# SitaoLuan/When-Do-GNNs-Help

Measured on AMD Instinct MI355X. Metric: aggregation edges/sec (whole job; + %HBM roofline of the SpMM kernel), higher is better.
Workload: dtype f32; 1 GPU; synthetic homophily sweep (data_synthesis/4000-equivalent): 10 h-levels x 5 seeds = 50 graphs/GPU/step, N=2000 nodes, k=10, F=500 fp32, C=5; step = batched D^-1(A+I)X aggregation + edge/label stati...; parallelism=independent sweep shards x1 (no data-path collective; job-table broadcast + r...

## Files before the change

when-do-gnns-help_amd/csrc/gemm.hip:

```cpp
#include "wdg_common.h"
#include "split_bf16.h"

namespace {

using namespace wdg;

typedef float f32x16 __attribute__((ext_vector_type(16)));

constexpr int BM = 128, BK = 16, THREADS = 256;
constexpr int LDA_S = BK + 1;

template <int NT>
__device__ __forceinline__ void tile_bias(global_ptr<const float> bias, int col0, int li, int N, float (&bv)[NT]) {
#pragma unroll
    for (int t = 0; t < NT; ++t) {
        const int gn = col0 + t * 32 + li;
        bv[t] = (bias && gn < N) ? bias[gn] : 0.f;
    }
}

template <int NT>
__device__ __forceinline__ void tile_store(const f32x16 (&acc)[NT], float (&bv)[NT], global_ptr<float> C, int64_t ldc, int row0,
                                           int col0, int li, int lk, int M, int N, int act) {
#pragma unroll
    for (int t = 0; t < NT; ++t) asm volatile("" : "+v"(bv[t]));
    const bool relu = act == WDG_ACT_RELU;
    const bool full = row0 + 32 <= M;
#pragma unroll
    for (int t = 0; t < NT; ++t) {
        const int gn = col0 + t * 32 + li;
        if (gn >= N) continue;
        global_ptr<float> p = C + static_cast<int64_t>(row0 + 4 * lk) * ldc + gn;
#pragma unroll
        for (int r = 0; r < 16; ++r) {
            float v = acc[t][r] + bv[t];
            if (relu) v = fmaxf(v, 0.f);
            if (full || row0 + (r & 3) + 8 * (r >> 2) + 4 * lk < M) *p = v;
            p += ((r & 3) == 3) ? 5 * ldc : ldc;
            if ((r & 3) == 3) __builtin_amdgcn_sched_barrier(0);
        }
    }
}

template <int NT, bool TRANSB>
__global__ __launch_bounds__(THREADS) void gemm_f32_kernel(const wdg_gemm_job *__restrict__ jobs,
                                                           const wdg_gemm_job inline_job) {
    constexpr int BN = 32 * NT;
    constexpr int LDB_S = TRANSB ? (BK + 1) : (BN + 1);
    __shared__ float As[BM * LDA_S];
    __shared__ float Bs[TRANSB ? BN * LDB_S : BK * LDB_S];

    const desc_ptr<wdg_gemm_job> job = descriptor(jobs, inline_job, blockIdx.z);
    const global_ptr<const float> A = to_global(job->A), B = to_global(job->B), bias = to_global(job->bias);
    const global_ptr<float> C = to_global(job->C);
    const int64_t lda = job->lda, ldb = job->ldb, ldc = job->ldc;
    const int M = job->M, N = job->N, K = job->K, act = job->act;
    const int tid = threadIdx.x, wave = tid >> 6, lane = tid & 63;
    const int m0 = blockIdx.x * BM, n0 = blockIdx.y * BN;
    if (m0 >= M || n0 >= N) return;
    const bool split = jobs == nullptr && gridDim.z > 1;
    int kb = 0, ke = K;
    global_ptr<float> Cw = C;
    if (split) {
        const int kc = (((K + static_cast<int>(gridDim.z) - 1) / static_cast<int>(gridDim.z)) + BK - 1) / BK * BK;
        kb = min(K, static_cast<int>(blockIdx.z) * kc), ke = min(K, kb + kc);
        Cw = C + static_cast<int64_t>(blockIdx.z) * M * ldc;
    }

    constexpr int A_PER = BM * BK / THREADS;
    constexpr int B_PER = BN * BK / THREADS;
    float ra[A_PER], rb[B_PER];

    auto load_tiles = [&](int k0) {
#pragma unroll
        for (int i = 0; i < A_PER; ++i) {
            const int e = tid + i * THREADS, k = e % BK, m = e / BK;
            const int gm = m0 + m, gk = k0 + k;
            ra[i] = (gm < M && gk < ke) ? A[static_cast<int64_t>(gm) * lda + gk] : 0.f;
        }
#pragma unroll
        for (int i = 0; i < B_PER; ++i) {
            const int e = tid + i * THREADS;
            if constexpr (TRANSB) {
                const int k = e % BK, n = e / BK;
                const int gn = n0 + n, gk = k0 + k;
                rb[i] = (gn < N && gk < ke) ? B[static_cast<int64_t>(gn) * ldb + gk] : 0.f;
            } else {
                const int n = e % BN, k = e / BN;
                const int gn = n0 + n, gk = k0 + k;
                rb[i] = (gn < N && gk < ke) ? B[static_cast<int64_t>(gk) * ldb + gn] : 0.f;
            }
        }
    };
    auto store_tiles = [&]() {
#pragma unroll
        for (int i = 0; i < A_PER; ++i) {
            const int e = tid + i * THREADS, k = e % BK, m = e / BK;
            As[m * LDA_S + k] = ra[i];
        }
#pragma unroll
        for (int i = 0; i < B_PER; ++i) {
            const int e = tid + i * THREADS;
            if constexpr (TRANSB) {
                const int k = e % BK, n = e / BK;
                Bs[n * LDB_S + k] = rb[i];
            } else {
                const int n = e % BN, k = e / BN;
                Bs[k * LDB_S + n] = rb[i];
            }
        }
    };

    f32x16 acc[NT];
#pragma unroll
    for (int t = 0; t < NT; ++t)
#pragma unroll
        for (int r = 0; r < 16; ++r) acc[t][r] = 0.f;

    const int li = lane & 31, lk = lane >> 5;
    float bv[NT];
    tile_bias<NT>(bias, n0, li, N, bv);
    load_tiles(kb);
    for (int k0 = kb; k0 < ke; k0 += BK) {
        __syncthreads();
        store_tiles();
        __syncthreads();
        if (k0 + BK < ke) load_tiles(k0 + BK);
#pragma unroll
        for (int kk = 0; kk < BK; kk += 2) {
            const float a = As[(wave * 32 + li) * LDA_S + kk + lk];
#pragma unroll
            for (int t = 0; t < NT; ++t) {
                float b;
                if constexpr (TRANSB) b = Bs[(t * 32 + li) * LDB_S + kk + lk];
                else b = Bs[(kk + lk) * LDB_S + t * 32 + li];
                acc[t] = __builtin_amdgcn_mfma_f32_32x32x2f32(a, b, acc[t], 0, 0, 0);
            }
        }
    }

    tile_store<NT>(acc, bv, Cw, ldc, m0 + wave * 32, n0, li, lk, M, N, act);
}

__global__ __launch_bounds__(256) void gemm_splitk_reduce(const float *__restrict__ P, int splits, int M, int N, int64_t ldp,
                                                          const float *__restrict__ bias, int act, float *__restrict__ C, int64_t ldc) {
    const int64_t i = static_cast<int64_t>(blockIdx.x) * 256 + threadIdx.x;
    if (i >= static_cast<int64_t>(M) * N) return;
    const int m = static_cast<int>(i / N), n = static_cast<int>(i % N);
    float v = P[static_cast<int64_t>(m) * ldp + n];
    for (int z = 1; z < splits; ++z) v += P[(static_cast<int64_t>(z) * M + m) * ldp + n];
    if (bias) v += bias[n];
    if (act == WDG_ACT_RELU) v = fmaxf(v, 0.f);
    C[static_cast<int64_t>(m) * ldc + n] = v;
}

constexpr int BRES_THREADS = 1024, BRES_COLS = 64;

struct BresGroup {
    f32x4_t r[4];
};

template <int NT, bool SWAP>
__device__ __forceinline__ void bres_compute(const BresGroup &grp, int kbase, int lk, int li, const float *Bres,
                                             f32x16 (&acc)[NT]) {
    float lo[8], hi[8];
#pragma unroll
    for (int j = 0; j < 4; ++j) {
        const auto xy = __builtin_amdgcn_permlane32_swap(__float_as_uint(grp.r[j].x), __float_as_uint(grp.r[j].y), false, false);
        const auto zw = __builtin_amdgcn_permlane32_swap(__float_as_uint(grp.r[j].z), __float_as_uint(grp.r[j].w), false, false);
        lo[2 * j] = __uint_as_float(xy[0]), hi[2 * j] = __uint_as_float(xy[1]);
        lo[2 * j + 1] = __uint_as_float(zw[0]), hi[2 * j + 1] = __uint_as_float(zw[1]);
    }
    constexpr int CH = 2, CHUNKS = 16 / CH;
    float bq[2][CH][NT];
    auto read_chunk = [&](int c, float (&dst)[CH][NT]) {
#pragma unroll
        for (int s = 0; s < CH; ++s) {
            const int row = kbase + 2 * (CH * c + s) + lk;
#pragma unroll
            for (int t = 0; t < NT; ++t) dst[s][t] = Bres[row * BRES_COLS + ((t * 32 + li) ^ (lk << 5))];
        }
    };
    read_chunk(0, bq[0]);
#pragma unroll
    for (int c = 0; c < CHUNKS; ++c) {
        if (c + 1 < CHUNKS) read_chunk(c + 1, bq[(c + 1) & 1]);
        __builtin_amdgcn_sched_barrier(0);
#pragma unroll
        for (int s = 0; s < CH; ++s) {
            const int h = CH * c + s;
            const float a = h < 8 ? lo[h] : hi[h - 8];
#pragma unroll
            for (int t = 0; t < NT; ++t)
                acc[t] = SWAP ? __builtin_amdgcn_mfma_f32_32x32x2f32(bq[c & 1][s][t], a, acc[t], 0, 0, 0)
                              : __builtin_amdgcn_mfma_f32_32x32x2f32(a, bq[c & 1][s][t], acc[t], 0, 0, 0);
        }
        __builtin_amdgcn_sched_barrier(0);
    }
}

__device__ __forceinline__ void bres_stage_b(global_ptr<const float> B, int64_t ldb, int K, int N, float *Bres) {
    const int k_rows = (K + 31) / 32 * 32;
    for (int base = threadIdx.x; base < k_rows * BRES_COLS; base += 8 * BRES_THREADS) {
        float v[8];
#pragma unroll
        for (int u = 0; u < 8; ++u) {
            const int idx = base + u * BRES_THREADS, k = idx / BRES_COLS, n = idx % BRES_COLS;
            v[u] = (k < K && n < N) ? B[static_cast<int64_t>(k) * ldb + n] : 0.f;
        }
#pragma unroll
        for (int u = 0; u < 8; ++u) {
            const int idx = base + u * BRES_THREADS, k = idx / BRES_COLS;
            if (idx < k_rows * BRES_COLS) Bres[idx ^ ((k & 1) << 5)] = v[u];
        }
    }
}

template <int NT, bool SWAP>
__device__ __forceinline__ void bres_tile(global_ptr<const float> a_lane, int K, int lk, int li, const float *Bres,
                                          f32x16 (&acc)[NT]) {
    const int full = K / 32;
    BresGroup g0, g1;
    auto load_group = [&](int g, BresGroup &dst) {
#pragma unroll
        for (int j = 0; j < 4; ++j) dst.r[j] = *(const global_ptr<const f32x4_t>)(a_lane + g * 32 + j * 4);
    };
    int g = 0;
    if (full > 0) load_group(0, g0);
    for (; g + 2 <= full; g += 2) {
        load_group(g + 1, g1);
        __builtin_amdgcn_sched_barrier(0);
        bres_compute<NT, SWAP>(g0, g * 32, lk, li, Bres, acc);
        __builtin_amdgcn_sched_barrier(0);
        load_group(min(g + 2, full - 1), g0);
        __builtin_amdgcn_sched_barrier(0);
        bres_compute<NT, SWAP>(g1, (g + 1) * 32, lk, li, Bres, acc);
        __builtin_amdgcn_sched_barrier(0);
    }
    if (g < full) bres_compute<NT, SWAP>(g0, g * 32, lk, li, Bres, acc), ++g;
    if (full * 32 < K) {
#pragma unroll
        for (int j = 0; j < 4; ++j) {
            const int k0 = full * 32 + 16 * lk + j * 4;
            g1.r[j] = f32x4_t{0.f, 0.f, 0.f, 0.f};
            if (k0 < K) g1.r[j] = *(const global_ptr<const f32x4_t>)(a_lane + full * 32 + j * 4);
        }
        bres_compute<NT, SWAP>(g1, full * 32, lk, li, Bres, acc);
    }
}

template <int NT>
__global__ __launch_bounds__(BRES_THREADS) void gemm_bres_kernel(const wdg_gemm_job *__restrict__ jobs,
                                                                   const wdg_gemm_job inline_job, int n_parts) {
    extern __shared__ float Bres[];
    const int job_id = blockIdx.x / n_parts, part = blockIdx.x % n_parts;
    const desc_ptr<wdg_gemm_job> job = descriptor(jobs, inline_job, job_id);
    const global_ptr<const float> A = to_global(job->A), B = to_global(job->B), bias = to_global(job->bias);
    const global_ptr<float> C = to_global(job->C);
    const int64_t lda = job->lda, ldb = job->ldb, ldc = job->ldc;
    const int M = job->M, N = job->N, K = job->K, act = job->act;
    const int wave = threadIdx.x >> 6, lane = threadIdx.x & 63, li = lane & 31, lk = lane >> 5;
    if (M <= 0 || N <= 0) return;
    bres_stage_b(B, ldb, K, N, Bres);
    __syncthreads();

    const int tiles = (M + 31) / 32, per_part = (tiles + n_parts - 1) / n_parts;
    const int t_end = min((part + 1) * per_part, tiles);
    for (int tile = part * per_part + wave; tile < t_end; tile += BRES_THREADS / 64) {
        const int gm = tile * 32 + li;
        const global_ptr<const float> a_lane = A + static_cast<int64_t>(gm < M ? gm : M - 1) * lda + 16 * lk;
        f32x16 acc[NT];
#pragma unroll
        for (int t = 0; t < NT; ++t)
#pragma unroll
            for (int r = 0; r < 16; ++r) acc[t][r] = 0.f;
        float bv[NT];
        tile_bias<NT>(bias, 0, li, N, bv);
        bres_tile<NT, false>(a_lane, K, lk, li, Bres, acc);
        tile_store<NT>(acc, bv, C, ldc, tile * 32, 0, li, lk, M, N, act);
    }
}

constexpr int MLP2_MAX_C = 8;

template <int NT>
__global__ __launch_bounds__(BRES_THREADS) void mlp2_bres_kernel(const wdg_mlp2_job *__restrict__ jobs, int n_parts) {
    extern __shared__ float Bres[];
    const int job_id = blockIdx.x / n_parts, part = blockIdx.x % n_parts;
    const desc_ptr<wdg_mlp2_job> job = (desc_ptr<wdg_mlp2_job>)(jobs + job_id);
    const global_ptr<const float> A = to_global(job->A), W0 = to_global(job->W0), b0 = to_global(job->b0);
    const global_ptr<const float> W1 = to_global(job->W1), b1 = to_global(job->b1);
    const global_ptr<float> Z = to_global(job->Z);
    const int64_t lda = job->lda, ldw0 = job->ldw0, ldw1 = job->ldw1, ldz = job->ldz;
    const int M = job->M, K = job->K, H = job->H, C = job->C, act = job->act;
    const int wave = threadIdx.x >> 6, lane = threadIdx.x & 63, li = lane & 31, lk = lane >> 5;
    if (M <= 0 || H <= 0 || C <= 0) return;
    float *const w1s = Bres + (K + 31) / 32 * 32 * BRES_COLS;
    float *const b0s = w1s + BRES_COLS * MLP2_MAX_C;
    bres_stage_b(W0, ldw0, K, H, Bres);
    for (int idx = threadIdx.x; idx < BRES_COLS * MLP2_MAX_C; idx += BRES_THREADS) {
        const int col = idx / MLP2_MAX_C, c = idx % MLP2_MAX_C;
        w1s[idx] = (col < H && c < C) ? W1[static_cast<int64_t>(col) * ldw1 + c] : 0.f;
    }
    if (threadIdx.x < BRES_COLS) b0s[threadIdx.x] = (b0 && threadIdx.x < H) ? b0[threadIdx.x] : 0.f;
    __syncthreads();

    const int tiles = (M + 31) / 32, per_part = (tiles + n_parts - 1) / n_parts;
    const int t_end = min((part + 1) * per_part, tiles);
    const bool relu = act == WDG_ACT_RELU;
    for (int tile = part * per_part + wave; tile < t_end; tile += BRES_THREADS / 64) {
        const int gm = tile * 32 + li;
        const global_ptr<const float> a_lane = A + static_cast<int64_t>(gm < M ? gm : M - 1) * lda + 16 * lk;
        f32x16 acc[NT];
#pragma unroll
        for (int t = 0; t < NT; ++t)
#pragma unroll
            for (int r = 0; r < 16; ++r) acc[t][r] = 0.f;
        bres_tile<NT, true>(a_lane, K, lk, li, Bres, acc);

        float z[MLP2_MAX_C];
#pragma unroll
        for (int c = 0; c < MLP2_MAX_C; ++c) z[c] = 0.f;
        int lds_off = lk * 4;
        asm volatile("" : "+v"(lds_off));
#pragma unroll
        for (int t = 0; t < NT; ++t) {
#pragma unroll
            for (int r4 = 0; r4 < 4; ++r4) {
                const int col0 = t * 32 + r4 * 8 + lds_off;
                const float4 bb = *reinterpret_cast<const float4 *>(b0s + col0);
                float h[4] = {acc[t][4 * r4] + bb.x, acc[t][4 * r4 + 1] + bb.y, acc[t][4 * r4 + 2] + bb.z, acc[t][4 * r4 + 3] + bb.w};
#pragma unroll
                for (int e = 0; e < 4; ++e) {
                    if (relu) h[e] = fmaxf(h[e], 0.f);
                    const float4 wa = *reinterpret_cast<const float4 *>(w1s + (col0 + e) * MLP2_MAX_C);
                    const float4 wb = *reinterpret_cast<const float4 *>(w1s + (col0 + e) * MLP2_MAX_C + 4);
                    z[0] = fmaf(h[e], wa.x, z[0]); z[1] = fmaf(h[e], wa.y, z[1]);
                    z[2] = fmaf(h[e], wa.z, z[2]); z[3] = fmaf(h[e], wa.w, z[3]);
                    z[4] = fmaf(h[e], wb.x, z[4]); z[5] = fmaf(h[e], wb.y, z[5]);
                    z[6] = fmaf(h[e], wb.z, z[6]); z[7] = fmaf(h[e], wb.w, z[7]);
                }
                __builtin_amdgcn_sched_barrier(0);
            }
        }
#pragma unroll
        for (int c = 0; c < MLP2_MAX_C; ++c) z[c] += __shfl_xor(z[c], 32);
        if (lk == 0 && gm < M) {
            const global_ptr<float> zp = Z + static_cast<int64_t>(gm) * ldz;
#pragma unroll
            for (int c = 0; c < MLP2_MAX_C; ++c)
                if (c < C) zp[c] = z[c] + (b1 ? b1[c] : 0.f);
        }
    }
}

constexpr int SPLIT_KQ = 128, SPLIT_KB = SPLIT_KQ / 8;
constexpr int SPLIT_PIECE_WORDS = SPLIT_KB * BRES_COLS * 4;
constexpr int SPLIT_BUF_WORDS = 3 * SPLIT_PIECE_WORDS;
static_assert(SPLIT_KB * BRES_COLS == BRES_THREADS, "one (k block, column) pair of a buffer per thread");

__device__ __forceinline__ void split_load_w(global_ptr<const float> W0, int64_t ldw0, int K, int H, int k0, float (&w)[8]) {
    int tid = threadIdx.x;
    asm volatile("" : "+v"(tid));
    const int col = tid % BRES_COLS, kb = tid / BRES_COLS;
    if (k0 + SPLIT_KQ <= K && H == BRES_COLS) {
        const global_ptr<const float> p = W0 + static_cast<int64_t>(k0 + 8 * kb) * ldw0 + col;
#pragma unroll
        for (int j = 0; j < 8; ++j) w[j] = p[j * ldw0];
        return;
    }
#pragma unroll
    for (int j = 0; j < 8; ++j) {
        const int k = k0 + 8 * kb + j;
        const float v = W0[static_cast<int64_t>(min(k, K - 1)) * ldw0 + min(col, H - 1)];
        w[j] = (k < K && col < H) ? v : 0.f;
    }
}
__device__ __forceinline__ void split_write_w(const float (&w)[8], unsigned *buf) {
    unsigned h[4], m[4], l[4];
#pragma unroll
    for (int j = 0; j < 4; ++j) split_pair(w[2 * j], w[2 * j + 1], h[j], m[j], l[j]);
    u32x4_t *dst = reinterpret_cast<u32x4_t *>(buf) + threadIdx.x;
    dst[0] = u32x4_t{h[0], h[1], h[2], h[3]};
    dst[SPLIT_PIECE_WORDS / 4] = u32x4_t{m[0], m[1], m[2], m[3]};
    dst[2 * (SPLIT_PIECE_WORDS / 4)] = u32x4_t{l[0], l[1], l[2], l[3]};
}

typedef float f32x4_acc __attribute__((ext_vector_type(4)));
struct SplitStep { f32x4_t a[2], b[2]; };

template <int NT16>
__device__ __forceinline__ void split_compute(const SplitStep &c, int kb, int n, const unsigned *Ws, f32x4_acc (&acc)[2][NT16]) {
    u32x4_t xh[2], xm[2], xl[2];
#pragma unroll
    for (int s = 0; s < 2; ++s) {
        unsigned ph[4], pm[4], pl[4];
        split_pair(c.a[s].x, c.a[s].y, ph[0], pm[0], pl[0]);
        split_pair(c.a[s].z, c.a[s].w, ph[1], pm[1], pl[1]);
        split_pair(c.b[s].x, c.b[s].y, ph[2], pm[2], pl[2]);
        split_pair(c.b[s].z, c.b[s].w, ph[3], pm[3], pl[3]);
        xh[s] = u32x4_t{ph[0], ph[1], ph[2], ph[3]}, xm[s] = u32x4_t{pm[0], pm[1], pm[2], pm[3]}, xl[s] = u32x4_t{pl[0], pl[1], pl[2], pl[3]};
    }
    const u32x4_t *wrow = reinterpret_cast<const u32x4_t *>(Ws) + kb * BRES_COLS + n;
#pragma unroll
    for (int T = 0; T < NT16; ++T) {
        const u32x4_t wl = wrow[T * 16 + 2 * (SPLIT_PIECE_WORDS / 4)];
        const u32x4_t wm = wrow[T * 16 + SPLIT_PIECE_WORDS / 4];
        const u32x4_t wh = wrow[T * 16];
#pragma unroll
        for (int s = 0; s < 2; ++s) {
            acc[s][T] = __builtin_amdgcn_mfma_f32_16x16x32_bf16(as_frag(wl), as_frag(xh[s]), acc[s][T], 0, 0, 0);
            acc[s][T] = __builtin_amdgcn_mfma_f32_16x16x32_bf16(as_frag(wm), as_frag(xm[s]), acc[s][T], 0, 0, 0);
            acc[s][T] = __builtin_amdgcn_mfma_f32_16x16x32_bf16(as_frag(wm), as_frag(xh[s]), acc[s][T], 0, 0, 0);
            acc[s][T] = __builtin_amdgcn_mfma_f32_16x16x32_bf16(as_frag(wh), as_frag(xl[s]), acc[s][T], 0, 0, 0);
            acc[s][T] = __builtin_amdgcn_mfma_f32_16x16x32_bf16(as_frag(wh), as_frag(xm[s]), acc[s][T], 0, 0, 0);
            acc[s][T] = __builtin_amdgcn_mfma_f32_16x16x32_bf16(as_frag(wh), as_frag(xh[s]), acc[s][T], 0, 0, 0);
        }
    }
}

template <int NT>
__global__ __launch_bounds__(BRES_THREADS) void mlp2_split_kernel(const wdg_mlp2_job *__restrict__ jobs, int n_parts) {
    constexpr int NT16 = 2 * NT;
    extern __shared__ float Bres[];
    const int job_id = blockIdx.x / n_parts, part = blockIdx.x % n_parts;
    const desc_ptr<wdg_mlp2_job> job = (desc_ptr<wdg_mlp2_job>)(jobs + job_id);
    const global_ptr<const float> A = to_global(job->A), W0 = to_global(job->W0), b0 = to_global(job->b0);
    const global_ptr<const float> W1 = to_global(job->W1), b1 = to_global(job->b1);
    const global_ptr<float> Z = to_global(job->Z);
    const int64_t lda = job->lda, ldw0 = job->ldw0, ldw1 = job->ldw1, ldz = job->ldz;
    const int64_t ags = job->a_group_stride > 0 ? job->a_group_stride : 16;
    const int M = job->M, K = job->K, H = job->H, C = job->C, act = job->act;
    const int wave = threadIdx.x >> 6, lane = threadIdx.x & 63, n = lane & 15, q = lane >> 4;
    if (M <= 0 || H <= 0 || C <= 0) return;
    unsigned *const Ws = reinterpret_cast<unsigned *>(Bres);
    float *const w1s = Bres + 2 * SPLIT_BUF_WORDS;
    float *const b0s = w1s + BRES_COLS * MLP2_MAX_C;
    for (int idx = threadIdx.x; idx < BRES_COLS * MLP2_MAX_C; idx += BRES_THREADS) {
        const int col = idx / MLP2_MAX_C, c = idx % MLP2_MAX_C;
        w1s[idx] = (col < H && c < C) ? W1[static_cast<int64_t>(col) * ldw1 + c] : 0.f;
    }
    if (threadIdx.x < BRES_COLS) b0s[threadIdx.x] = (b0 && threadIdx.x < H) ? b0[threadIdx.x] : 0.f;

    const int tiles = (M + 31) / 32, per_part = (tiles + n_parts - 1) / n_parts;
    const int t_first = part * per_part, t_end = min((part + 1) * per_part, tiles);
    const bool relu = act == WDG_ACT_RELU;
    const int steps = (K + 31) / 32, quarters = (K + SPLIT_KQ - 1) / SPLIT_KQ;
    for (int t0 = t_first; t0 < t_end; t0 += BRES_THREADS / 64) {
        const int tile = t0 + wave;
        const bool have = tile < t_end;
        global_ptr<const float> a_row[2];
#pragma unroll
        for (int s = 0; s < 2; ++s) {
            const int gm = tile * 32 + 16 * s + n;
            a_row[s] = A + static_cast<int64_t>(have && gm < M ? gm : M - 1) * lda + (q >> 1) * ags + (q & 1) * 8;
        }
        f32x4_acc acc[2][NT16];
#pragma unroll
        for (int s = 0; s < 2; ++s)
#pragma unroll
            for (int T = 0; T < NT16; ++T) acc[s][T] = f32x4_acc{0.f, 0.f, 0.f, 0.f};
        auto load_step = [&](int st, SplitStep &dst) {
            st = min(st, steps - 1);
            if (32 * st + 32 <= K) {
#pragma unroll
                for (int s = 0; s < 2; ++s) {
                    dst.a[s] = *(const global_ptr<const f32x4_t>)(a_row[s] + 2 * ags * st);
                    dst.b[s] = *(const global_ptr<const f32x4_t>)(a_row[s] + 2 * ags * st + 4);
                }
                return;
            }
            const int k = 32 * st + 8 * q;
            const f32x4_t zero{0.f, 0.f, 0.f, 0.f};
#pragma unroll
            for (int s = 0; s < 2; ++s) {
                const global_ptr<const float> row0 = a_row[s] - ((q >> 1) * ags + (q & 1) * 8);
                const int ka = min(k, K - 4), kb = min(k + 4, K - 4);
                const f32x4_t va = *(const global_ptr<const f32x4_t>)(row0 + (ka >> 4) * ags + (ka & 15));
                const f32x4_t vb = *(const global_ptr<const f32x4_t>)(row0 + (kb >> 4) * ags + (kb & 15));
                dst.a[s] = k < K ? va : zero;
                dst.b[s] = k + 4 < K ? vb : zero;
            }
        };
        SplitStep sa, sb;
        float w[8];
        load_step(0, sa);
        split_load_w(W0, ldw0, K, H, 0, w);
        split_write_w(w, Ws);
        __syncthreads();
        for (int qu = 0; qu < quarters; ++qu) {
            const unsigned *cur = Ws + (qu & 1) * SPLIT_BUF_WORDS;
            if (qu + 1 < quarters) split_load_w(W0, ldw0, K, H, (qu + 1) * SPLIT_KQ, w);
            if (have) {
#pragma unroll
                for (int c = 0; c < 4; c += 2) {
                    const int base = 4 * qu + c;
                    if (base >= steps) break;
                    load_step(base + 1, sb);
                    __builtin_amdgcn_sched_barrier(0);
                    split_compute<NT16>(sa, 4 * c + q, n, cur, acc);
                    __builtin_amdgcn_sched_barrier(0);
                    load_step(base + 2, sa);
                    __builtin_amdgcn_sched_barrier(0);
                    if (base + 1 < steps) split_compute<NT16>(sb, 4 * c + 4 + q, n, cur, acc);
                    __builtin_amdgcn_sched_barrier(0);
                }
            }
            if (qu + 1 < quarters) split_write_w(w, Ws + ((qu + 1) & 1) * SPLIT_BUF_WORDS);
            __syncthreads();
        }
        if (!have) continue;

        int lds_off = q * 4;
        asm volatile("" : "+v"(lds_off));
#pragma unroll
        for (int s = 0; s < 2; ++s) {
            float z[MLP2_MAX_C];
#pragma unroll
            for (int c = 0; c < MLP2_MAX_C; ++c) z[c] = 0.f;
#pragma unroll
            for (int T = 0; T < NT16; ++T) {
                const int col0 = 16 * T + lds_off;
                const float4 bb = *reinterpret_cast<const float4 *>(b0s + col0);
                float h[4] = {acc[s][T][0] + bb.x, acc[s][T][1] + bb.y, acc[s][T][2] + bb.z, acc[s][T][3] + bb.w};
#pragma unroll
                for (int e = 0; e < 4; ++e) {
                    if (relu) h[e] = fmaxf(h[e], 0.f);
                    const float4 wa = *reinterpret_cast<const float4 *>(w1s + (col0 + e) * MLP2_MAX_C);
                    const float4 wb = *reinterpret_cast<const float4 *>(w1s + (col0 + e) * MLP2_MAX_C + 4);
                    z[0] = fmaf(h[e], wa.x, z[0]); z[1] = fmaf(h[e], wa.y, z[1]);
                    z[2] = fmaf(h[e], wa.z, z[2]); z[3] = fmaf(h[e], wa.w, z[3]);
                    z[4] = fmaf(h[e], wb.x, z[4]); z[5] = fmaf(h[e], wb.y, z[5]);
                    z[6] = fmaf(h[e], wb.z, z[6]); z[7] = fmaf(h[e], wb.w, z[7]);
                }
                __builtin_amdgcn_sched_barrier(0);
            }
#pragma unroll
            for (int c = 0; c < MLP2_MAX_C; ++c) {
                z[c] += __shfl_xor(z[c], 16);
                z[c] += __shfl_xor(z[c], 32);
            }
            const int gm = tile * 32 + 16 * s + n;
            if (q == 0 && gm < M) {
                const global_ptr<float> zp = Z + static_cast<int64_t>(gm) * ldz;
#pragma unroll
                for (int c = 0; c < MLP2_MAX_C; ++c)
                    if (c < C) zp[c] = z[c] + (b1 ? b1[c] : 0.f);
            }
        }
    }
}

bool bres_shape_ok(int n_jobs, int max_M, int max_N, int K) {
    if (!(max_N <= BRES_COLS && K > 0 && K % 4 == 0 && ceil_div(K, 32) * 32 * BRES_COLS * 4 <= 128 * 1024)) return false;
    if (getenv("WDG_GEMM_TILE")) return false;
    if (getenv("WDG_GEMM_RESIDENT")) return true;
    return static_cast<int64_t>(n_jobs) * ceil_div(max_M, BM) >= 3 * std::max(wdg_device_cus(), 8);
}

int bres_parts(int n_jobs, int max_M) {
    const int tiles = static_cast<int>(ceil_div(max_M, 32));
    const int cus = std::max(wdg_device_cus(), 8);
    int parts = 1;
    int64_t best = INT64_MAX;
    for (int p = 1; p <= 16 && (p == 1 || tiles / p >= 8); ++p) {
        const int64_t cost = ceil_div(static_cast<int64_t>(n_jobs) * p, cus) * ceil_div(ceil_div(tiles, p), BRES_THREADS / 64);
        if (cost < best) best = cost, parts = p;
    }
    return parts;
}

int launch_bres(const wdg_gemm_job *jobs, const wdg_gemm_job &inl, int n_jobs, int max_M, int max_N, int K, hipStream_t st) {
    static thread_local int configured_dev = -1;
    if (configured_dev != current_device()) {
        for (const void *k : {reinterpret_cast<const void *>(gemm_bres_kernel<1>), reinterpret_cast<const void *>(gemm_bres_kernel<2>)})
            if (hipFuncSetAttribute(k, hipFuncAttributeMaxDynamicSharedMemorySize, 128 * 1024) != hipSuccess)
                return fail(WDG_ERR_LAUNCH, "hipFuncSetAttribute(max dynamic LDS) failed");
        configured_dev = wdg::current_device();
    }
    const int parts = bres_parts(n_jobs, max_M);
    const size_t lds = static_cast<size_t>(ceil_div(K, 32) * 32) * BRES_COLS * 4;
    const dim3 grid(static_cast<unsigned>(n_jobs) * parts);
    if (max_N > 32) hipLaunchKernelGGL(gemm_bres_kernel<2>, grid, dim3(BRES_THREADS), lds, st, jobs, inl, parts);
    else hipLaunchKernelGGL(gemm_bres_kernel<1>, grid, dim3(BRES_THREADS), lds, st, jobs, inl, parts);
    return check_launch("gemm_bres_kernel");
}

constexpr int SK_THREADS = 256, SK_KCHUNK = 2048, SK_N = 8;

template <int NCOLS>
__global__ __launch_bounds__(256) void gemm_skinny_wave_kernel(const float *__restrict__ A, int64_t lda, const float *__restrict__ B,
                                                                 int64_t ldb, const float *__restrict__ bias, int act,
                                                                 float *__restrict__ C, int64_t ldc, int M, int K) {
    const int lane = threadIdx.x & 63, row = blockIdx.x * 4 + (threadIdx.x >> 6);
    if (row >= M) return;
    const float *a = A + static_cast<int64_t>(row) * lda;
    float acc[NCOLS];
#pragma unroll
    for (int c = 0; c < NCOLS; ++c) acc[c] = 0.f;
#pragma unroll 4
    for (int k = lane; k < K; k += 64) {
        const float av = a[k];
        const float *b = B + static_cast<int64_t>(k) * ldb;
#pragma unroll
        for (int c = 0; c < NCOLS; ++c) acc[c] = fmaf(av, b[c], acc[c]);
    }
#pragma unroll
    for (int c = 0; c < NCOLS; ++c)
        for (int o = 32; o > 0; o >>= 1) acc[c] += __shfl_xor(acc[c], o);
    if (lane == 0) {
        float *out = C + static_cast<int64_t>(row) * ldc;
#pragma unroll
        for (int c = 0; c < NCOLS; ++c) {
            const float v = acc[c] + (bias ? bias[c] : 0.f);
            out[c] = act == WDG_ACT_RELU ? fmaxf(v, 0.f) : v;
        }
    }
}

template <int LPR>
__global__ __launch_bounds__(SK_THREADS) void gemm_skinny_kernel(const float *__restrict__ A, int64_t lda, const float *__restrict__ B,
                                                                 int64_t ldb, const float *__restrict__ bias, int act,
                                                                 float *__restrict__ C, int64_t ldc, int M, int N, int K) {
    __shared__ float Bs[SK_KCHUNK * SK_N];
    constexpr int ROWS = SK_THREADS / LPR;
    const int tid = threadIdx.x, gl = tid % LPR;
    const int row = blockIdx.x * ROWS + tid / LPR;
    const float *a = A + static_cast<int64_t>(min(row, M - 1)) * lda;
    float acc[SK_N];
#pragma unroll
    for (int c = 0; c < SK_N; ++c) acc[c] = 0.f;
    for (int k0 = 0; k0 < K; k0 += SK_KCHUNK) {
        const int kc = min(SK_KCHUNK, K - k0);
        if (k0) __syncthreads();
#pragma unroll 8
        for (int i = tid; i < kc * SK_N; i += SK_THREADS) {
            const int k = i >> 3, c = i & 7;
            Bs[i] = c < N ? B[static_cast<int64_t>(k0 + k) * ldb + c] : 0.f;
        }
        __syncthreads();
#pragma unroll 8
        for (int k = gl; k < kc; k += LPR) {
            const float av = a[k0 + k];
            const float4 b0 = *reinterpret_cast<const float4 *>(&Bs[k * SK_N]), b1 = *reinterpret_cast<const float4 *>(&Bs[k * SK_N + 4]);
            acc[0] = fmaf(av, b0.x, acc[0]), acc[1] = fmaf(av, b0.y, acc[1]), acc[2] = fmaf(av, b0.z, acc[2]), acc[3] = fmaf(av, b0.w, acc[3]);
            acc[4] = fmaf(av, b1.x, acc[4]), acc[5] = fmaf(av, b1.y, acc[5]), acc[6] = fmaf(av, b1.z, acc[6]), acc[7] = fmaf(av, b1.w, acc[7]);
        }
    }
#pragma unroll
    for (int c = 0; c < SK_N; ++c)
        for (int o = LPR / 2; o > 0; o >>= 1) acc[c] += __shfl_xor(acc[c], o);
    if (gl == 0 && row < M) {
        float *out = C + static_cast<int64_t>(row) * ldc;
#pragma unroll
        for (int c = 0; c < SK_N; ++c) {
            if (c >= N) break;
            const float v = acc[c] + (bias ? bias[c] : 0.f);
            out[c] = act == WDG_ACT_RELU ? fmaxf(v, 0.f) : v;
        }
    }
}

}

extern "C" {

int wdg_gemm_f32(const float *A, int64_t lda, const float *B, int64_t ldb, int transb, const float *bias, int act,
                 float *C, int64_t ldc, int32_t M, int32_t N, int32_t K, wdg_stream_t stream) {
    WDG_REQUIRE(M >= 0 && N >= 0 && K >= 0, "gemm: negative size");
    if (M == 0 || N == 0) return WDG_OK;
    WDG_REQUIRE(A && B && C, "gemm: null matrix");
    WDG_REQUIRE(lda >= K && ldc >= N && ldb >= (transb ? K : N), "gemm: leading dimension too small");
    WDG_REQUIRE(act == WDG_ACT_NONE || act == WDG_ACT_RELU, "gemm: bad activation");
    hipStream_t st = wdg::as_stream(stream);
    if (!transb && (reinterpret_cast<uintptr_t>(A) & 15) == 0 && lda % 4 == 0 && bres_shape_ok(1, M, N, K)) {
        wdg_gemm_job jb{};
        jb.A = A; jb.B = B; jb.bias = bias; jb.C = C;
        jb.lda = lda; jb.ldb = ldb; jb.ldc = ldc;
        jb.M = M; jb.N = N; jb.K = K; jb.act = act;
        return launch_bres(nullptr, jb, 1, M, N, K, st);
    }
    const bool wide = N > 32;
    const dim3 grid(static_cast<unsigned>(wdg::ceil_div(M, BM)), static_cast<unsigned>(wdg::ceil_div(N, wide ? 64 : 32)));
    wdg_gemm_job j{};
    j.A = A; j.B = B; j.bias = bias; j.C = C;
    j.lda = lda; j.ldb = ldb; j.ldc = ldc;
    j.M = M; j.N = N; j.K = K; j.act = act;
    const wdg_gemm_job *none = nullptr;
    if (wide) {
        if (transb) hipLaunchKernelGGL((gemm_f32_kernel<2, true>), grid, dim3(THREADS), 0, st, none, j);
        else hipLaunchKernelGGL((gemm_f32_kernel<2, false>), grid, dim3(THREADS), 0, st, none, j);
    } else {
        if (transb) hipLaunchKernelGGL((gemm_f32_kernel<1, true>), grid, dim3(THREADS), 0, st, none, j);
        else hipLaunchKernelGGL((gemm_f32_kernel<1, false>), grid, dim3(THREADS), 0, st, none, j);
    }
    return wdg::check_launch("gemm_f32_kernel");
}

int32_t wdg_gemm_splitk_plan(int32_t M, int32_t N, int32_t K) {
    if (const char *e = getenv("WDG_GEMM_SPLITK")) {
        const int v = atoi(e);
        if (v >= 0 && v <= 16) return std::max(v, 1);
    }
    const int cus = std::max(wdg_device_cus(), 8);
    const int64_t tiles = wdg::ceil_div(M, BM) * wdg::ceil_div(N, N > 32 ? 64 : 32);
    if (M <= 0 || N <= 0 || tiles * 2 > cus || K < 1024) return 1;
    return static_cast<int32_t>(std::max<int64_t>(1, std::min<int64_t>({cus / tiles, K / 256, 16})));
}

size_t wdg_gemm_splitk_workspace_bytes(int32_t M, int32_t N, int32_t splits) {
    return static_cast<size_t>(std::max(splits, 1)) * std::max(M, 0) * ((std::max(N, 0) + 3) / 4 * 4) * sizeof(float) + 256;
}

int wdg_gemm_splitk_f32(const float *A, int64_t lda, const float *B, int64_t ldb, const float *bias, int act, float *C, int64_t ldc,
                        int32_t M, int32_t N, int32_t K, int32_t splits, void *workspace, size_t workspace_bytes, wdg_stream_t stream) {
    WDG_REQUIRE(M >= 0 && N >= 0 && K >= 0, "gemm_splitk: negative size");
    WDG_REQUIRE(splits >= 1 && splits <= 16, "gemm_splitk: 1 .. 16 splits");
    if (M == 0 || N == 0) return WDG_OK;
    if (splits == 1 || K < splits * BK) return wdg_gemm_f32(A, lda, B, ldb, 0, bias, act, C, ldc, M, N, K, stream);
    WDG_REQUIRE(A && B && C, "gemm_splitk: null matrix");
    WDG_REQUIRE(lda >= K && ldc >= N && ldb >= N, "gemm_splitk: leading dimension too small");
    WDG_REQUIRE(act == WDG_ACT_NONE || act == WDG_ACT_RELU, "gemm_splitk: bad activation");
    if (!workspace || workspace_bytes < wdg_gemm_splitk_workspace_bytes(M, N, splits))
        return wdg::fail(WDG_ERR_WORKSPACE, "gemm_splitk: workspace too small");
    hipStream_t st = wdg::as_stream(stream);
    float *P = reinterpret_cast<float *>((reinterpret_cast<uintptr_t>(workspace) + 255) & ~static_cast<uintptr_t>(255));
    const int64_t ldp = (N + 3) / 4 * 4;
    const bool wide = N > 32;
    const dim3 grid(static_cast<unsigned>(wdg::ceil_div(M, BM)), static_cast<unsigned>(wdg::ceil_div(N, wide ? 64 : 32)), static_cast<unsigned>(splits));
    wdg_gemm_job j{};
    j.A = A; j.B = B; j.bias = nullptr; j.C = P;
    j.lda = lda; j.ldb = ldb; j.ldc = ldp;
    j.M = M; j.N = N; j.K = K; j.act = WDG_ACT_NONE;
    const wdg_gemm_job *none = nullptr;
    if (wide) hipLaunchKernelGGL((gemm_f32_kernel<2, false>), grid, dim3(THREADS), 0, st, none, j);
    else hipLaunchKernelGGL((gemm_f32_kernel<1, false>), grid, dim3(THREADS), 0, st, none, j);
    hipLaunchKernelGGL(gemm_splitk_reduce, dim3(static_cast<unsigned>(wdg::ceil_div(static_cast<int64_t>(M) * N, 256))), dim3(256), 0, st, P, splits,
                       M, N, ldp, bias, act, C, ldc);
    return wdg::check_launch("gemm_splitk");
}

int wdg_gemm_skinny_f32(const float *A, int64_t lda, const float *B, int64_t ldb, const float *bias, int act, float *C, int64_t ldc,
                        int32_t M, int32_t N, int32_t K, wdg_stream_t stream) {
    WDG_REQUIRE(M >= 0 && N >= 0 && K >= 0, "gemm_skinny: negative size");
    WDG_REQUIRE(N <= SK_N, "gemm_skinny: more than 8 columns (wdg_gemm_f32 takes those)");
    if (M == 0 || N == 0) return WDG_OK;
    WDG_REQUIRE(A && B && C, "gemm_skinny: null matrix");
    WDG_REQUIRE(lda >= K && ldc >= N && ldb >= N, "gemm_skinny: leading dimension too small");
    WDG_REQUIRE(act == WDG_ACT_NONE || act == WDG_ACT_RELU, "gemm_skinny: bad activation");
    hipStream_t st = wdg::as_stream(stream);
    if (K <= 16)
        hipLaunchKernelGGL(gemm_skinny_kernel<1>, dim3(static_cast<unsigned>(wdg::ceil_div(M, SK_THREADS))), dim3(SK_THREADS), 0, st, A, lda,
                           B, ldb, bias, act, C, ldc, M, N, K);
    else if (K <= 128)
        hipLaunchKernelGGL(gemm_skinny_kernel<4>, dim3(static_cast<unsigned>(wdg::ceil_div(M, SK_THREADS / 4))), dim3(SK_THREADS), 0, st, A,
                           lda, B, ldb, bias, act, C, ldc, M, N, K);
    else if (K <= 512)
        hipLaunchKernelGGL(gemm_skinny_kernel<16>, dim3(static_cast<unsigned>(wdg::ceil_div(M, SK_THREADS / 16))), dim3(SK_THREADS), 0, st, A,
                           lda, B, ldb, bias, act, C, ldc, M, N, K);
    else {
        const dim3 grid(static_cast<unsigned>(wdg::ceil_div(M, 4)));
#define WDG_SKINNY_WAVE(NC) hipLaunchKernelGGL(gemm_skinny_wave_kernel<NC>, grid, dim3(256), 0, st, A, lda, B, ldb, bias, act, C, ldc, M, K)
        switch (N) {
            case 1: WDG_SKINNY_WAVE(1); break;
            case 2: WDG_SKINNY_WAVE(2); break;
            case 3: WDG_SKINNY_WAVE(3); break;
            case 4: WDG_SKINNY_WAVE(4); break;
            case 5: WDG_SKINNY_WAVE(5); break;
            case 6: WDG_SKINNY_WAVE(6); break;
            case 7: WDG_SKINNY_WAVE(7); break;
            default: WDG_SKINNY_WAVE(8); break;
        }
#undef WDG_SKINNY_WAVE
    }
    return wdg::check_launch("gemm_skinny_kernel");
}

int wdg_gemm_batched_flags_f32(const wdg_gemm_job *jobs_dev, int32_t n_jobs, int32_t max_M, int32_t max_N, int32_t max_K,
                               uint32_t flags, wdg_stream_t stream) {
    WDG_REQUIRE(n_jobs >= 0 && max_M >= 0 && max_N >= 0 && max_K >= 0, "gemm_batched: negative size");
    if (n_jobs == 0 || max_M == 0 || max_N == 0) return WDG_OK;
    WDG_REQUIRE(jobs_dev != nullptr, "gemm_batched: null job table");
    WDG_REQUIRE(n_jobs <= 65535, "gemm_batched: more than 65535 jobs per launch");
    if ((flags & WDG_GEMM_A_VEC4) && bres_shape_ok(n_jobs, max_M, max_N, max_K))
        return launch_bres(jobs_dev, wdg_gemm_job{}, n_jobs, max_M, max_N, max_K, wdg::as_stream(stream));
    const bool wide = max_N > 32;
    const dim3 grid(static_cast<unsigned>(wdg::ceil_div(max_M, BM)), static_cast<unsigned>(wdg::ceil_div(max_N, wide ? 64 : 32)),
                    static_cast<unsigned>(n_jobs));
    if (wide) hipLaunchKernelGGL((gemm_f32_kernel<2, false>), grid, dim3(THREADS), 0, wdg::as_stream(stream), jobs_dev, wdg_gemm_job{});
    else hipLaunchKernelGGL((gemm_f32_kernel<1, false>), grid, dim3(THREADS), 0, wdg::as_stream(stream), jobs_dev, wdg_gemm_job{});
    return wdg::check_launch("gemm_f32_kernel (batched)");
}

int wdg_gemm_batched_f32(const wdg_gemm_job *jobs_dev, int32_t n_jobs, int32_t max_M, int32_t max_N,
                         wdg_stream_t stream) {
    return wdg_gemm_batched_flags_f32(jobs_dev, n_jobs, max_M, max_N, 0, 0, stream);
}

int wdg_mlp2_batched_f32(const wdg_mlp2_job *jobs_dev, int32_t n_jobs, int32_t max_M, int32_t max_K, int32_t max_H,
                         int32_t max_C, wdg_stream_t stream) {
    return wdg_mlp2_batched_flags_f32(jobs_dev, n_jobs, max_M, max_K, max_H, max_C, 0u, stream);
}

int wdg_mlp2_batched_flags_f32(const wdg_mlp2_job *jobs_dev, int32_t n_jobs, int32_t max_M, int32_t max_K, int32_t max_H,
                               int32_t max_C, uint32_t flags, wdg_stream_t stream) {
    WDG_REQUIRE((flags & ~(WDG_KERNEL_SPLIT | WDG_KERNEL_CHAIN | WDG_OPERAND_TILED)) == 0 &&
                    (flags & (WDG_KERNEL_SPLIT | WDG_KERNEL_CHAIN)) != (WDG_KERNEL_SPLIT | WDG_KERNEL_CHAIN), "mlp2_batched: bad flags");
    WDG_REQUIRE(n_jobs >= 0 && max_M >= 0 && max_K >= 0 && max_H >= 0 && max_C >= 0, "mlp2_batched: negative size");
    if (n_jobs == 0 || max_M == 0 || max_H == 0 || max_C == 0) return WDG_OK;
    WDG_REQUIRE(jobs_dev != nullptr, "mlp2_batched: null job table");
    if (max_H > BRES_COLS || max_C > MLP2_MAX_C || max_K <= 0 || max_K % 4 != 0 ||
        wdg::ceil_div(max_K, 32) * 32 * BRES_COLS * 4 > 128 * 1024)
        return wdg::fail(WDG_ERR_UNSUPPORTED, "mlp2_batched: needs H <= 64, C <= 8, 0 < K <= 512, K % 4 == 0 (use two wdg_gemm calls)");
    WDG_REQUIRE(static_cast<int64_t>(n_jobs) * 16 <= 0x7fffffffLL, "mlp2_batched: too many jobs");
    const size_t lds_max = 128 * 1024 + (BRES_COLS * MLP2_MAX_C + BRES_COLS) * sizeof(float);
    static thread_local int configured_dev = -1;
    if (configured_dev != wdg::current_device()) {
        for (const void *k : {reinterpret_cast<const void *>(mlp2_bres_kernel<1>), reinterpret_cast<const void *>(mlp2_bres_kernel<2>)})
            if (hipFuncSetAttribute(k, hipFuncAttributeMaxDynamicSharedMemorySize, static_cast<int>(lds_max)) != hipSuccess)
                return wdg::fail(WDG_ERR_LAUNCH, "hipFuncSetAttribute(max dynamic LDS) failed");
        configured_dev = wdg::current_device();
    }
    const int parts = bres_parts(n_jobs, max_M);
    const dim3 grid(static_cast<unsigned>(n_jobs) * parts);
    hipStream_t st = wdg::as_stream(stream);
    bool split = (flags & WDG_KERNEL_CHAIN) == 0;
    if (!(flags & (WDG_KERNEL_SPLIT | WDG_KERNEL_CHAIN)))
        if (const char *e = getenv("WDG_MLP2_SPLIT")) split = atoi(e) != 0;
    if (!split && (flags & WDG_OPERAND_TILED))
        return wdg::fail(WDG_ERR_UNSUPPORTED, "mlp2_batched: the fp32-chain kernel reads row-major A only (the table holds a tiled A)");
    {
        if (split) {
            const size_t lds_split = (2 * SPLIT_BUF_WORDS + BRES_COLS * MLP2_MAX_C + BRES_COLS) * sizeof(float);
            static thread_local int split_dev = -1;
            if (split_dev != wdg::current_device()) {
                for (const void *k : {reinterpret_cast<const void *>(mlp2_split_kernel<1>), reinterpret_cast<const void *>(mlp2_split_kernel<2>)})
                    if (hipFuncSetAttribute(k, hipFuncAttributeMaxDynamicSharedMemorySize, static_cast<int>(lds_split)) != hipSuccess)
                        return wdg::fail(WDG_ERR_LAUNCH, "hipFuncSetAttribute(max dynamic LDS) failed");
                split_dev = wdg::current_device();
            }
            if (max_H > 32) hipLaunchKernelGGL(mlp2_split_kernel<2>, grid, dim3(BRES_THREADS), lds_split, st, jobs_dev, parts);
            else hipLaunchKernelGGL(mlp2_split_kernel<1>, grid, dim3(BRES_THREADS), lds_split, st, jobs_dev, parts);
            return wdg::check_launch("mlp2_split_kernel");
        }
    }
    const size_t lds = (static_cast<size_t>(wdg::ceil_div(max_K, 32) * 32) * BRES_COLS + BRES_COLS * MLP2_MAX_C + BRES_COLS) * sizeof(float);
    if (max_H > 32) hipLaunchKernelGGL(mlp2_bres_kernel<2>, grid, dim3(BRES_THREADS), lds, st, jobs_dev, parts);
    else hipLaunchKernelGGL(mlp2_bres_kernel<1>, grid, dim3(BRES_THREADS), lds, st, jobs_dev, parts);
    return wdg::check_launch("mlp2_bres_kernel");
}

}
```

Before: 18.01 billion edges/s.

## Restructure split-bf16 MLP2 kernel loop: peel K tail, wave-uniform W loads, hoist b1

Result: faster. 18.65 billion edges/s (median of 6 runs) (+3.6%).

```diff
diff --git a/when-do-gnns-help_amd/csrc/gemm.hip b/when-do-gnns-help_amd/csrc/gemm.hip
--- a/when-do-gnns-help_amd/csrc/gemm.hip
+++ b/when-do-gnns-help_amd/csrc/gemm.hip
@@ -359,28 +359,25 @@
 constexpr int SPLIT_BUF_WORDS = 3 * SPLIT_PIECE_WORDS;
 static_assert(SPLIT_KB * BRES_COLS == BRES_THREADS, "one (k block, column) pair of a buffer per thread");
 
-__device__ __forceinline__ void split_load_w(global_ptr<const float> W0, int64_t ldw0, int K, int H, int k0, float (&w)[8]) {
-    int tid = threadIdx.x;
-    asm volatile("" : "+v"(tid));
-    const int col = tid % BRES_COLS, kb = tid / BRES_COLS;
-    if (k0 + SPLIT_KQ <= K && H == BRES_COLS) {
-        const global_ptr<const float> p = W0 + static_cast<int64_t>(k0 + 8 * kb) * ldw0 + col;
-#pragma unroll
-        for (int j = 0; j < 8; ++j) w[j] = p[j * ldw0];
-        return;
-    }
+__device__ __forceinline__ void split_load_w(global_ptr<const float> W0, int64_t ldw0, int K, int H, int k0, int wave, int lane, float (&w)[8]) {
+    unsigned at = static_cast<unsigned>(min(lane, H - 1)) * 4u;
+    asm volatile("" : "+v"(at));
 #pragma unroll
     for (int j = 0; j < 8; ++j) {
-        const int k = k0 + 8 * kb + j;
-        const float v = W0[static_cast<int64_t>(min(k, K - 1)) * ldw0 + min(col, H - 1)];
-        w[j] = (k < K && col < H) ? v : 0.f;
-    }
-}
-__device__ __forceinline__ void split_write_w(const float (&w)[8], unsigned *buf) {
+        const global_ptr<const float> row = W0 + static_cast<int64_t>(min(k0 + 8 * wave + j, K - 1)) * ldw0;
+        w[j] = *(global_ptr<const float>)((global_ptr<const char>)row + at);
+    }
+}
+__device__ __forceinline__ void split_write_w(float (&w)[8], int K, int H, int k0, int wave, int lane, unsigned *buf) {
+#pragma unroll
+    for (int j = 0; j < 8; ++j) {
+        asm volatile("" : "+v"(w[j]));
+        w[j] = (k0 + 8 * wave + j < K && lane < H) ? w[j] : 0.f;
+    }
     unsigned h[4], m[4], l[4];
 #pragma unroll
     for (int j = 0; j < 4; ++j) split_pair(w[2 * j], w[2 * j + 1], h[j], m[j], l[j]);
-    u32x4_t *dst = reinterpret_cast<u32x4_t *>(buf) + threadIdx.x;
+    u32x4_t *dst = reinterpret_cast<u32x4_t *>(buf) + wave * BRES_COLS + lane;
     dst[0] = u32x4_t{h[0], h[1], h[2], h[3]};
     dst[SPLIT_PIECE_WORDS / 4] = u32x4_t{m[0], m[1], m[2], m[3]};
     dst[2 * (SPLIT_PIECE_WORDS / 4)] = u32x4_t{l[0], l[1], l[2], l[3]};
@@ -431,7 +428,8 @@
     const int64_t lda = job->lda, ldw0 = job->ldw0, ldw1 = job->ldw1, ldz = job->ldz;
     const int64_t ags = job->a_group_stride > 0 ? job->a_group_stride : 16;
     const int M = job->M, K = job->K, H = job->H, C = job->C, act = job->act;
-    const int wave = threadIdx.x >> 6, lane = threadIdx.x & 63, n = lane & 15, q = lane >> 4;
+    const int wave = __builtin_amdgcn_readfirstlane(threadIdx.x >> 6);
+    const int lane = threadIdx.x & 63, n = lane & 15, q = lane >> 4;
     if (M <= 0 || H <= 0 || C <= 0) return;
     unsigned *const Ws = reinterpret_cast<unsigned *>(Bres);
     float *const w1s = Bres + 2 * SPLIT_BUF_WORDS;
@@ -445,15 +443,28 @@
     const int tiles = (M + 31) / 32, per_part = (tiles + n_parts - 1) / n_parts;
     const int t_first = part * per_part, t_end = min((part + 1) * per_part, tiles);
     const bool relu = act == WDG_ACT_RELU;
-    const int steps = (K + 31) / 32, quarters = (K + SPLIT_KQ - 1) / SPLIT_KQ;
+    const int whole = K / 32, quarters = (K + SPLIT_KQ - 1) / SPLIT_KQ;
+    const unsigned *const last = Ws + ((quarters - 1) & 1) * SPLIT_BUF_WORDS;
     for (int t0 = t_first; t0 < t_end; t0 += BRES_THREADS / 64) {
         const int tile = t0 + wave;
-        const bool have = tile < t_end;
+        float w[8];
+        split_load_w(W0, ldw0, K, H, 0, wave, lane, w);
+        if (tile >= t_end) {
+            split_write_w(w, K, H, 0, wave, lane, Ws);
+            __syncthreads();
+            for (int qu = 1; qu < quarters; ++qu) {
+                split_load_w(W0, ldw0, K, H, qu * SPLIT_KQ, wave, lane, w);
+                split_write_w(w, K, H, qu * SPLIT_KQ, wave, lane, Ws + (qu & 1) * SPLIT_BUF_WORDS);
+                __syncthreads();
+            }
+            __syncthreads();
+            continue;
+        }
         global_ptr<const float> a_row[2];
 #pragma unroll
         for (int s = 0; s < 2; ++s) {
             const int gm = tile * 32 + 16 * s + n;
-            a_row[s] = A + static_cast<int64_t>(have && gm < M ? gm : M - 1) * lda + (q >> 1) * ags + (q & 1) * 8;
+            a_row[s] = A + static_cast<int64_t>(gm < M ? gm : M - 1) * lda + (q >> 1) * ags + (q & 1) * 8;
         }
         f32x4_acc acc[2][NT16];
 #pragma unroll
@@ -461,61 +472,64 @@
 #pragma unroll
             for (int T = 0; T < NT16; ++T) acc[s][T] = f32x4_acc{0.f, 0.f, 0.f, 0.f};
         auto load_step = [&](int st, SplitStep &dst) {
-            st = min(st, steps - 1);
-            if (32 * st + 32 <= K) {
-#pragma unroll
-                for (int s = 0; s < 2; ++s) {
-                    dst.a[s] = *(const global_ptr<const f32x4_t>)(a_row[s] + 2 * ags * st);
-                    dst.b[s] = *(const global_ptr<const f32x4_t>)(a_row[s] + 2 * ags * st + 4);
+            st = min(st, whole - 1);
+#pragma unroll
+            for (int s = 0; s < 2; ++s) {
+                dst.a[s] = *(const global_ptr<const f32x4_t>)(a_row[s] + 2 * ags * st);
+                dst.b[s] = *(const global_ptr<const f32x4_t>)(a_row[s] + 2 * ags * st + 4);
+            }
+        };
+        SplitStep sa, sb;
+        if (whole > 0) load_step(0, sa);
+        split_write_w(w, K, H, 0, wave, lane, Ws);
+        __syncthreads();
+        if (whole > 0) {
+            for (int qu = 0;; ++qu) {
+                const unsigned *cur = Ws + (qu & 1) * SPLIT_BUF_WORDS;
+                split_load_w(W0, ldw0, K, H, (qu + 1) * SPLIT_KQ, wave, lane, w);
+#pragma unroll
+                for (int c = 0; c < 4; c += 2) {
+                    const int base = 4 * qu + c;
+                    load_step(base + 1, sb);
+                    __builtin_amdgcn_sched_barrier(0);
+                    if (base < whole) split_compute<NT16>(sa, 4 * c + q, n, cur, acc);
+                    __builtin_amdgcn_sched_barrier(0);
+                    load_step(base + 2, sa);
+                    __builtin_amdgcn_sched_barrier(0);
+                    if (base + 1 < whole) split_compute<NT16>(sb, 4 * c + 4 + q, n, cur, acc);
+                    __builtin_amdgcn_sched_barrier(0);
                 }
-                return;
-            }
-            const int k = 32 * st + 8 * q;
+                if (qu + 1 == quarters) break;
+                split_write_w(w, K, H, (qu + 1) * SPLIT_KQ, wave, lane, Ws + ((qu + 1) & 1) * SPLIT_BUF_WORDS);
+                __syncthreads();
+            }
+        }
+        if (32 * whole < K) {
+            int qo = q;
+            asm volatile("" : "+v"(qo));
+            const int k = 32 * whole + 8 * qo;
             const f32x4_t zero{0.f, 0.f, 0.f, 0.f};
 #pragma unroll
             for (int s = 0; s < 2; ++s) {
-                const global_ptr<const float> row0 = a_row[s] - ((q >> 1) * ags + (q & 1) * 8);
+                const global_ptr<const float> row0 = a_row[s] - ((qo >> 1) * ags + (qo & 1) * 8);
                 const int ka = min(k, K - 4), kb = min(k + 4, K - 4);
                 const f32x4_t va = *(const global_ptr<const f32x4_t>)(row0 + (ka >> 4) * ags + (ka & 15));
                 const f32x4_t vb = *(const global_ptr<const f32x4_t>)(row0 + (kb >> 4) * ags + (kb & 15));
-                dst.a[s] = k < K ? va : zero;
-                dst.b[s] = k + 4 < K ? vb : zero;
-            }
-        };
-        SplitStep sa, sb;
-        float w[8];
-        load_step(0, sa);
-        split_load_w(W0, ldw0, K, H, 0, w);
-        split_write_w(w, Ws);
-        __syncthreads();
-        for (int qu = 0; qu < quarters; ++qu) {
-            const unsigned *cur = Ws + (qu & 1) * SPLIT_BUF_WORDS;
-            if (qu + 1 < quarters) split_load_w(W0, ldw0, K, H, (qu + 1) * SPLIT_KQ, w);
-            if (have) {
-#pragma unroll
-                for (int c = 0; c < 4; c += 2) {
-                    const int base = 4 * qu + c;
-                    if (base >= steps) break;
-                    load_step(base + 1, sb);
-                    __builtin_amdgcn_sched_barrier(0);
-                    split_compute<NT16>(sa, 4 * c + q, n, cur, acc);
-                    __builtin_amdgcn_sched_barrier(0);
-                    load_step(base + 2, sa);
-                    __builtin_amdgcn_sched_barrier(0);
-                    if (base + 1 < steps) split_compute<NT16>(sb, 4 * c + 4 + q, n, cur, acc);
-                    __builtin_amdgcn_sched_barrier(0);
-                }
-            }
-            if (qu + 1 < quarters) split_write_w(w, Ws + ((qu + 1) & 1) * SPLIT_BUF_WORDS);
-            __syncthreads();
-        }
-        if (!have) continue;
-
+                sb.a[s] = k < K ? va : zero;
+                sb.b[s] = k + 4 < K ? vb : zero;
+            }
+            split_compute<NT16>(sb, 4 * (whole & 3) + q, n, last, acc);
+        }
         int lds_off = q * 4;
         asm volatile("" : "+v"(lds_off));
+        int b1_at = n & (MLP2_MAX_C - 1);
+        asm volatile("" : "+v"(b1_at));
+        float b1v = 0.f;
+        if (b1) b1v = b1[static_cast<unsigned>(min(b1_at, C - 1))];
+        float zs[2][MLP2_MAX_C];
 #pragma unroll
         for (int s = 0; s < 2; ++s) {
-            float z[MLP2_MAX_C];
+            float (&z)[MLP2_MAX_C] = zs[s];
 #pragma unroll
             for (int c = 0; c < MLP2_MAX_C; ++c) z[c] = 0.f;
 #pragma unroll
@@ -540,14 +554,19 @@
                 z[c] += __shfl_xor(z[c], 16);
                 z[c] += __shfl_xor(z[c], 32);
             }
+        }
+        asm volatile("" : "+v"(b1v));
+#pragma unroll
+        for (int s = 0; s < 2; ++s) {
             const int gm = tile * 32 + 16 * s + n;
             if (q == 0 && gm < M) {
                 const global_ptr<float> zp = Z + static_cast<int64_t>(gm) * ldz;
 #pragma unroll
                 for (int c = 0; c < MLP2_MAX_C; ++c)
-                    if (c < C) zp[c] = z[c] + (b1 ? b1[c] : 0.f);
-            }
-        }
+                    if (c < C) zp[c] = zs[s][c] + __int_as_float(__builtin_amdgcn_readlane(__float_as_int(b1v), c));
+            }
+        }
+        __syncthreads();
     }
 }
 
```
